# fpgasystems/GPU-FPGA-Recommendation-System

Measured on AMD Instinct MI355X. Metric: inferences/sec at batch 256, higher is better.
Workload: dtype f32; 1 GPU; Model-A (embedding_47_krnl: 47 tables, 1.415 GB) batch=256, fp32 FC 352-1024-512-256-1, all tables resident in one GPU's HBM; hash-filled tables, uniform per-table indices; index rows resident in HBM when the timed region starts (1024 rotating buffers), scores left in HBM (the bench contract's definition of `value`); value_pcie_inclusive = the reference's own loop (cuda_server.c:460-461,494-495): ; batch=256, driver_threads=2, workers_per_thread=2, batches_per_launch=64, parallelism=replicas x1

## Files before the change

### gpu-fpga-recommendation-system_amd/csrc/fr_fused.hip

```cpp
#include "fr_device.h"

constexpr int FR_FT_LD = 33;

template <int NT, int D>
__device__ __forceinline__ void ft_load_a(float4 (&r)[D][NT], const float4 *__restrict__ aq, int N, int g) {
#pragma unroll
    for (int i = 0; i < D; i++)
#pragma unroll
        for (int t = 0; t < NT; t++) r[i][t] = aq[(size_t)(2 * (g + i)) * N + 32 * t];
}

template <int NT, int D>
__device__ __forceinline__ void ft_compute(f32x16 (&acc)[NT], f32x16 &alt, const float4 (&r)[D][NT], const uint4 *bl, int gb) {
    uint4 rb[D];
#pragma unroll
    for (int i = 0; i < D; i++) rb[i] = bl[(size_t)(2 * (gb + i)) * FR_FT_LD];
    __builtin_amdgcn_sched_barrier(0);
#pragma unroll
    for (int i = 0; i < D; i++) {
        const float bx = __uint_as_float(rb[i].x), by = __uint_as_float(rb[i].y), bz = __uint_as_float(rb[i].z), bw = __uint_as_float(rb[i].w);
        if constexpr (NT == 1) {
            acc[0] = __builtin_amdgcn_mfma_f32_32x32x2f32(r[i][0].x, bx, acc[0], 0, 0, 0);
            alt = __builtin_amdgcn_mfma_f32_32x32x2f32(r[i][0].y, by, alt, 0, 0, 0);
            acc[0] = __builtin_amdgcn_mfma_f32_32x32x2f32(r[i][0].z, bz, acc[0], 0, 0, 0);
            alt = __builtin_amdgcn_mfma_f32_32x32x2f32(r[i][0].w, bw, alt, 0, 0, 0);
        } else {
#pragma unroll
            for (int t = 0; t < NT; t++) acc[t] = __builtin_amdgcn_mfma_f32_32x32x2f32(r[i][t].x, bx, acc[t], 0, 0, 0);
#pragma unroll
            for (int t = 0; t < NT; t++) acc[t] = __builtin_amdgcn_mfma_f32_32x32x2f32(r[i][t].y, by, acc[t], 0, 0, 0);
#pragma unroll
            for (int t = 0; t < NT; t++) acc[t] = __builtin_amdgcn_mfma_f32_32x32x2f32(r[i][t].z, bz, acc[t], 0, 0, 0);
#pragma unroll
            for (int t = 0; t < NT; t++) acc[t] = __builtin_amdgcn_mfma_f32_32x32x2f32(r[i][t].w, bw, acc[t], 0, 0, 0);
        }
    }
    __builtin_amdgcn_sched_barrier(0);
}

struct FtW {
    __amdgpu_buffer_rsrc_t rs;
    unsigned voff;
    unsigned row2;
};
__device__ __forceinline__ FtW ft_w(const float4 *wq, int K, int N, int hk, int lm) {
    FtW w;
    w.rs = __builtin_amdgcn_make_buffer_rsrc(const_cast<float4 *>(wq), 0, (unsigned)(K / 4) * (unsigned)N * 16u, 0x00020000);
    w.voff = (unsigned)(hk * N + lm) * 16u;
    w.row2 = 2u * (unsigned)N * 16u;
    return w;
}
__device__ __forceinline__ float4 ft_wload(const FtW &w, unsigned soff, int imm) {
    const u32x4 v = __builtin_amdgcn_raw_buffer_load_b128(w.rs, w.voff + imm, soff, 0);
    return make_float4(__uint_as_float(v.x), __uint_as_float(v.y), __uint_as_float(v.z), __uint_as_float(v.w));
}

template <int NT, int R, int CNT>
__device__ __forceinline__ void ft_ring_fill(float4 (&ring)[R][NT], const FtW &w, int n0, int g0) {
    const unsigned s0 = (unsigned)g0 * w.row2 + (unsigned)n0 * 16u;
#pragma unroll
    for (int g = 0; g < R && g < CNT; g++)
#pragma unroll
        for (int t = 0; t < NT; t++) ring[g][t] = ft_wload(w, s0 + (unsigned)g * w.row2, 512 * t);
    __builtin_amdgcn_sched_barrier(0);
}

template <int NT, int R, int CNT>
__device__ __forceinline__ void ft_gemm_ct(f32x16 (&acc)[NT], float4 (&ring)[R][NT], const FtW &w, int n0, const uint4 *Bq, int gb0, int g0, int hk,
                                           int lm) {
    const unsigned s0 = (unsigned)g0 * w.row2 + (unsigned)n0 * 16u;
    unsigned so = s0 + (unsigned)R * w.row2;
    const uint4 *bl = Bq + (size_t)(2 * gb0 + hk) * FR_FT_LD + lm;
    f32x16 alt;
#pragma unroll
    for (int i = 0; i < 16; i++) alt[i] = 0.0f;
    uint4 bcur = bl[0];
#pragma unroll
    for (int g = 0; g < CNT; g++) {
        const uint4 bnext = bl[(size_t)(2 * ((g + 1 < CNT) ? g + 1 : g)) * FR_FT_LD];
        const float bx = __uint_as_float(bcur.x), by = __uint_as_float(bcur.y), bz = __uint_as_float(bcur.z), bw = __uint_as_float(bcur.w);
        const float4(&a4)[NT] = ring[g % R];
        if constexpr (NT == 1) {
            acc[0] = __builtin_amdgcn_mfma_f32_32x32x2f32(a4[0].x, bx, acc[0], 0, 0, 0);
            alt = __builtin_amdgcn_mfma_f32_32x32x2f32(a4[0].y, by, alt, 0, 0, 0);
            acc[0] = __builtin_amdgcn_mfma_f32_32x32x2f32(a4[0].z, bz, acc[0], 0, 0, 0);
            alt = __builtin_amdgcn_mfma_f32_32x32x2f32(a4[0].w, bw, alt, 0, 0, 0);
        } else {
#pragma unroll
            for (int t = 0; t < NT; t++) acc[t] = __builtin_amdgcn_mfma_f32_32x32x2f32(a4[t].x, bx, acc[t], 0, 0, 0);
#pragma unroll
            for (int t = 0; t < NT; t++) acc[t] = __builtin_amdgcn_mfma_f32_32x32x2f32(a4[t].y, by, acc[t], 0, 0, 0);
#pragma unroll
            for (int t = 0; t < NT; t++) acc[t] = __builtin_amdgcn_mfma_f32_32x32x2f32(a4[t].z, bz, acc[t], 0, 0, 0);
#pragma unroll
            for (int t = 0; t < NT; t++) acc[t] = __builtin_amdgcn_mfma_f32_32x32x2f32(a4[t].w, bw, acc[t], 0, 0, 0);
        }
        if (g + R < CNT) {
#pragma unroll
            for (int t = 0; t < NT; t++) ring[g % R][t] = ft_wload(w, so, 512 * t);
            so += w.row2;
            asm volatile("" : "+s"(so));
        }
        __builtin_amdgcn_sched_barrier(0);
        bcur = bnext;
    }
    if constexpr (NT == 1) {
#pragma unroll
        for (int i = 0; i < 16; i++) acc[0][i] += alt[i];
    }
}

template <int NT, int D>
__device__ __forceinline__ void ft_gemm(f32x16 (&acc)[NT], const float4 *__restrict__ wq, int N, int n0, const uint4 *Bq, int gb0, int g0,
                                        int cnt, int hk, int lm) {
    const float4 *aq = wq + (size_t)hk * N + n0 + lm;
    const uint4 *bl = Bq + hk * FR_FT_LD + lm;
    float4 ra[D][NT], na[D][NT];
    f32x16 alt;
#pragma unroll
    for (int i = 0; i < 16; i++) alt[i] = 0.0f;
    const int nblk = cnt / D;
    ft_load_a<NT, D>(ra, aq, N, g0);
    for (int blk = 0; blk < nblk; blk++) {
        const int nx = (blk + 1 < nblk) ? (blk + 1) : blk;
        ft_load_a<NT, D>(na, aq, N, g0 + nx * D);
        ft_compute<NT, D>(acc, alt, ra, bl, gb0 + blk * D);
#pragma unroll
        for (int i = 0; i < D; i++)
#pragma unroll
            for (int t = 0; t < NT; t++) ra[i][t] = na[i][t];
    }
    if constexpr (NT == 1) {
#pragma unroll
        for (int i = 0; i < 16; i++) acc[0][i] += alt[i];
    }
}

__device__ __forceinline__ void ft_store_tile(uint4 *img, const f32x16 &acc, int n_local, int hk, int lm) {
#pragma unroll
    for (int i = 0; i < 4; i++) {
        uint4 v;
        v.x = __float_as_uint(acc[4 * i + 0]);
        v.y = __float_as_uint(acc[4 * i + 1]);
        v.z = __float_as_uint(acc[4 * i + 2]);
        v.w = __float_as_uint(acc[4 * i + 3]);
        img[(size_t)((n_local >> 2) + 2 * i + hk) * FR_FT_LD + lm] = v;
    }
}

template <int NB, int IPT, typename Sink>
__device__ __forceinline__ bool ft_gather_tile(const FrFusedArgs &a, const FrFusedBatch &bt, int m0, int wl, int ig, Sink &&sink) {
    uint64_t base[NB];
    uint32_t stride[NB], rows[NB], icol[NB];
    bool dense[NB];
#pragma unroll
    for (int p = 0; p < NB; p++) {
        const int w = 64 * p + wl < a.n_words ? 64 * p + wl : a.n_words - 1;
        const uint4 d0 = reinterpret_cast<const uint4 *>(a.words)[2 * w];
        const uint4 d1 = reinterpret_cast<const uint4 *>(a.words)[2 * w + 1];
        dense[p] = (d0.w & FR_DESC_DENSE) != 0;
        base[p] = (dense[p] ? (uint64_t)reinterpret_cast<uintptr_t>(bt.dense) : 0ull) + (((uint64_t)d0.y << 32) | d0.x);
        stride[p] = d0.z, rows[p] = d1.x, icol[p] = dense[p] ? 0u : d0.w * 4u;
    }
    const __amdgpu_buffer_rsrc_t rs_idx = __builtin_amdgcn_make_buffer_rsrc(const_cast<int32_t *>(bt.idx), 0, (unsigned)bt.batch * (unsigned)a.idx_stride * 4u, 0x00020000);
    uint32_t id[NB][IPT];
#pragma unroll
    for (int p = 0; p < NB; p++)
#pragma unroll
        for (int i = 0; i < IPT; i++)
            id[p][i] = (uint32_t)__builtin_amdgcn_raw_buffer_load_b32(rs_idx, (unsigned)(m0 + IPT * ig + i) * (unsigned)a.idx_stride * 4u + icol[p], 0, 0);
    bool bad = false;
    uint4 v[NB][IPT];
    auto load_rows = [&](int p) {
#pragma unroll
        for (int i = 0; i < IPT; i++) {
            const unsigned m = (unsigned)(m0 + IPT * ig + i);
            uint32_t r = id[p][i];
            const bool oob = !dense[p] & (r >= rows[p]);
            bad |= oob;
            r = oob ? 0u : r;
            r = dense[p] ? (m < (unsigned)bt.batch ? m : 0u) : r;
            typedef const u32x4_t __attribute__((address_space(1))) * gptr_t;
            const u32x4_t q = *(gptr_t)(base[p] + (uint64_t)r * stride[p]);
            v[p][i] = make_uint4(q.x, q.y, q.z, q.w);
        }
    };
    load_rows(0);
#pragma unroll
    for (int p = 0; p < NB; p++) {
        if (p + 1 < NB) load_rows(p + 1);
        const int w = 64 * p + wl;
        if (w < a.n_words) {
#pragma unroll
            for (int i = 0; i < IPT; i++) sink(w, i, (m0 + IPT * ig + i < bt.batch) ? v[p][i] : make_uint4(0u, 0u, 0u, 0u));
        }
    }
    return bad;
}

template <int T2W, int KG, int WPE, bool DB>
__global__ void __launch_bounds__(512, WPE) fr_fused_tile_kernel(const FrFusedArgs a) {
    extern __shared__ uint4 lds[];
    constexpr int RD = (WPE == 2) ? 1 : 2;
    const int KQ = a.K / 4;
    uint4 *Xq = lds;
    uint4 *R1b[2] = {Xq + (size_t)KQ * FR_FT_LD, Xq + (size_t)(KQ + (DB ? 64 : 0)) * FR_FT_LD};
    uint4 *R2 = lds;
    uint4 *R3 = DB ? lds + (size_t)(a.H2 / 4) * FR_FT_LD : lds;
    const int tid = threadIdx.x, lane = tid & 63;
    const int wave = __builtin_amdgcn_readfirstlane(tid >> 6);
    const int hk = lane >> 5, lm = lane & 31;
    const int bi = blockIdx.x / a.tiles_per_batch, tile = blockIdx.x - bi * a.tiles_per_batch;
    const FrFusedBatch &bt = a.b[bi];
    const int m0 = tile * 32;
    if (m0 >= bt.batch) return;
    int n_st = 0;
    auto stamp = [&]() {
        if (a.stamps && tid == 0 && n_st < 14) {
            a.stamps[16ull * blockIdx.x + n_st] = __builtin_amdgcn_s_memrealtime();
            if (n_st == 1) a.stamps[16ull * blockIdx.x + 14] = __builtin_amdgcn_s_memtime();
            if (n_st == 11) a.stamps[16ull * blockIdx.x + 15] = __builtin_amdgcn_s_memtime();
        }
        n_st++;
    };
    auto wstamp = [&](int k) {
        if (a.stamps && lane == 0) a.stamps[16ull * gridDim.x + (8ull * blockIdx.x + wave) * 4 + k] = __builtin_amdgcn_s_memrealtime();
    };
    stamp();
    const FtW W1 = ft_w(a.w1q, a.K, a.H1, hk, lm), W2 = ft_w(a.w2q, a.H1, a.H2, hk, lm), W3 = ft_w(a.w3q, a.H2, a.H3, hk, lm);
    constexpr int RA = 16 / RD, RB = 24 / T2W / RD;
    constexpr int KG1 = KG > 0 ? KG : 1;
    float4 ring1[RA][1];
    if constexpr (KG > 0) ft_ring_fill<1, RA, KG1>(ring1, W1, 32 * wave, 0);

    if constexpr (KG > 0) {
        const int wl = tid & 63, ig = tid >> 6;
        constexpr int NB = (2 * KG1 + 63) / 64;
        const bool bad = ft_gather_tile<NB, 4>(a, bt, m0, wl, ig, [&](int w, int i, const uint4 &x) { Xq[(size_t)w * FR_FT_LD + 4 * ig + i] = x; });
        if (bad) atomicOr_system(a.err_flag, 1);
    } else {
        const int wl = tid & 63, ig = tid >> 6;
        bool bad = false;
        for (int w0 = 0; w0 < a.n_words; w0 += 64) {
            const int w = w0 + wl;
            if (w < a.n_words) {
                const uint4 d0 = reinterpret_cast<const uint4 *>(a.words)[2 * w];
                const uint4 d1 = reinterpret_cast<const uint4 *>(a.words)[2 * w + 1];
                const uint64_t src = ((uint64_t)d0.y << 32) | d0.x;
                const uint32_t stride = d0.z, idx_col = d0.w, rows = d1.x;
                const bool is_dense = (idx_col & FR_DESC_DENSE) != 0;
                const char *base = is_dense ? reinterpret_cast<const char *>(bt.dense) + src : reinterpret_cast<const char *>(src);
                uint32_t id[4];
#pragma unroll
                for (int i = 0; i < 4; i++) {
                    const int m = m0 + 4 * ig + i;
                    id[i] = 0;
                    if (m < bt.batch) id[i] = is_dense ? (uint32_t)m : (uint32_t)bt.idx[(size_t)m * a.idx_stride + idx_col];
                    if (!is_dense && id[i] >= rows) {
                        bad = true;
                        id[i] = 0;
                    }
                }
                uint4 v[4];
#pragma unroll
                for (int i = 0; i < 4; i++) v[i] = *reinterpret_cast<const uint4 *>(base + (uint64_t)id[i] * stride);
#pragma unroll
                for (int i = 0; i < 4; i++)
                    Xq[(size_t)w * FR_FT_LD + 4 * ig + i] = (m0 + 4 * ig + i < bt.batch) ? v[i] : make_uint4(0u, 0u, 0u, 0u);
            }
        }
        if (bad) atomicOr_system(a.err_flag, 1);
    }
    __syncthreads();
    stamp();

    f32x16 acc2[T2W];
#pragma unroll
    for (int t = 0; t < T2W; t++)
#pragma unroll
        for (int i = 0; i < 16; i++) acc2[t][i] = 0.0f;
    const int n_chunks = a.H1 / 256;
    for (int c = 0; c < n_chunks; c++) {
        f32x16 acc1[1];
#pragma unroll
        for (int i = 0; i < 16; i++) acc1[0][i] = 0.0f;
        if constexpr (KG > 0) ft_gemm_ct<1, RA, KG1>(acc1, ring1, W1, c * 256 + 32 * wave, Xq, 0, 0, hk, lm);
        else ft_gemm<1, 4>(acc1, a.w1q, a.H1, c * 256 + 32 * wave, Xq, 0, 0, a.K / 8, hk, lm);
        stamp();
        if (c == 1) wstamp(0);
        if (c == 2) wstamp(3);
        float4 ring2[RB][T2W];
        ft_ring_fill<T2W, RB, 32>(ring2, W2, 32 * T2W * wave, 32 * c);
        uint4 *R1 = R1b[c & 1];
        if (!DB && c > 0) __syncthreads();
        ft_store_tile(R1, acc1[0], 32 * wave, hk, lm);
        __syncthreads();
        stamp();
        if (c == 1) wstamp(1);
        ft_gemm_ct<T2W, RB, 32>(acc2, ring2, W2, 32 * T2W * wave, R1, 0, 32 * c, hk, lm);
        if (c == 1) wstamp(2);
        if constexpr (KG > 0) {
            const int cn = (c + 1 < n_chunks) ? c + 1 : c;
            ft_ring_fill<1, RA, KG1>(ring1, W1, cn * 256 + 32 * wave, 0);
        }
    }
    float4 ring3[RA][1];
    ft_ring_fill<1, RA, 32 * T2W>(ring3, W3, 32 * wave, 0);
    __syncthreads();
#pragma unroll
    for (int t = 0; t < T2W; t++) ft_store_tile(R2, acc2[t], 32 * (T2W * wave + t), hk, lm);
    __syncthreads();
    stamp();

    f32x16 acc3[1];
#pragma unroll
    for (int i = 0; i < 16; i++) acc3[0][i] = 0.0f;
    ft_gemm_ct<1, RA, 32 * T2W>(acc3, ring3, W3, 32 * wave, R2, 0, 0, hk, lm);
    if (!DB) __syncthreads();
    ft_store_tile(R3, acc3[0], 32 * wave, hk, lm);
    __syncthreads();
    stamp();
    {
        const int il = tid & 31, sl = tid >> 5;
        const int rows_per = (a.H3 / 4) / 16;
        float s = 0.0f;
        for (int q = sl * rows_per; q < (sl + 1) * rows_per; q++) {
            const uint4 r = R3[(size_t)q * FR_FT_LD + il];
            const float4 w4 = reinterpret_cast<const float4 *>(a.wout)[q];
            s = fmaf(w4.x, __uint_as_float(r.x), s);
            s = fmaf(w4.y, __uint_as_float(r.y), s);
            s = fmaf(w4.z, __uint_as_float(r.z), s);
            s = fmaf(w4.w, __uint_as_float(r.w), s);
        }
        float *part = reinterpret_cast<float *>(R3 + (size_t)64 * FR_FT_LD);
        part[sl * 32 + il] = s;
        __syncthreads();
        if (tid < 32 && m0 + tid < bt.batch) {
            float t = part[tid];
#pragma unroll
            for (int i = 1; i < 16; i++) t += part[i * 32 + tid];
            bt.scores[m0 + tid] = t;
        }
    }
    stamp();
}

size_t frk_fused_lds_bytes(int K, int H2, int wpe) {
    if (wpe == 4) {
        const size_t phase1 = (size_t)(K / 4) + 64, phase2 = (size_t)(H2 / 4) > 68 ? (size_t)(H2 / 4) : 68;
        return (phase1 > phase2 ? phase1 : phase2) * FR_FT_LD * 16;
    }
    const size_t phase1 = (size_t)(K / 4) + 128;
    const size_t phase2 = (size_t)(H2 / 4) + 64 + 4;
    return (phase1 > phase2 ? phase1 : phase2) * FR_FT_LD * 16;
}

bool frk_fused_ok(int K, int H1, int H2, int H3) {
    const bool straight = (K == 352 || K == 880) && H2 == 512;
    if ((!straight && K % 32) || H1 % 256 || (H2 != 256 && H2 != 512) || H3 != 256) return false;
    return frk_fused_lds_bytes(K, H2, 4) <= 160 * 1024;
}

static int fused_wpe(int K, int H2) {
#ifdef FR_EXPERIMENTS
    const int forced = FR_KNOB_ONCE("FUSED_WPE", 0);
    if (forced == 2 || forced == 4) return forced == 4 && frk_fused_lds_bytes(K, H2, 4) > 80 * 1024 ? 2 : forced;
#endif
    return frk_fused_lds_bytes(K, H2, 4) <= 80 * 1024 ? 4 : 2;
}

template <int T2W, int KG, int WPE, bool DB>
static int fused_launch_inst(const FrFusedArgs &a, dim3 grid, size_t lds, hipStream_t s) {
    static FrLdsAttrOnce lds_once;
    if (int rc_ = fr_allow_full_lds(&fr_fused_tile_kernel<T2W, KG, WPE, DB>, lds_once)) return rc_;
    fr_fused_tile_kernel<T2W, KG, WPE, DB><<<grid, dim3(512), lds, s>>>(a);
    fr_note_kernel("fr_fused_tile_kernel<%d, %d, %d, %s>", T2W, KG, WPE, DB ? "true" : "false");
    KCHECK();
    return FR_OK;
}

int frk_fused_launch(const FrFusedArgs &a, hipStream_t s) {
    int wpe = fused_wpe(a.K, a.H2);
    const bool db = wpe == 2 && frk_fused_lds_bytes(a.K, a.H2, 2) <= 160 * 1024;
    const size_t lds = frk_fused_lds_bytes(a.K, a.H2, db ? 2 : 4);
    dim3 grid(a.n_batches * a.tiles_per_batch);
    if (a.H2 == 512) {
        if (a.K == 352) {
#ifdef FR_EXPERIMENTS
            if (wpe != 4) return fused_launch_inst<2, 44, 2, true>(a, grid, lds, s);
#endif
            return fused_launch_inst<2, 44, 4, false>(a, grid, lds, s);
        }
        if (a.K == 880) return fused_launch_inst<2, 110, 2, false>(a, grid, lds, s);
        if (db) return fused_launch_inst<2, 0, 2, true>(a, grid, lds, s);
        return fused_launch_inst<2, 0, 2, false>(a, grid, lds, s);
    }
    if (db) return fused_launch_inst<1, 0, 2, true>(a, grid, lds, s);
    return fused_launch_inst<1, 0, 2, false>(a, grid, lds, s);
}

constexpr int FR_M2_LD = 65;

template <int NT, int MT, int R, int CNT>
__device__ __forceinline__ void ftm_gemm_ct(f32x16 (&acc)[NT][MT], float4 (&ring)[R][NT], const FtW &w, int n0, const uint4 *Bq, int gb0, int g0, int hk,
                                            int lm) {
    const unsigned s0 = (unsigned)g0 * w.row2 + (unsigned)n0 * 16u;
    const uint4 *bl = Bq + (size_t)(2 * gb0 + hk) * FR_M2_LD + lm;
    uint4 bcur[MT];
#pragma unroll
    for (int mt = 0; mt < MT; mt++) bcur[mt] = bl[32 * mt];
    f32x16 alt[MT];
    if constexpr (NT == 1) {
#pragma unroll
        for (int mt = 0; mt < MT; mt++)
#pragma unroll
            for (int i = 0; i < 16; i++) alt[mt][i] = 0.0f;
    }
#pragma unroll
    for (int g = 0; g < CNT; g++) {
        uint4 bnext[MT];
        const int gn = (g + 1 < CNT) ? g + 1 : g;
#pragma unroll
        for (int mt = 0; mt < MT; mt++) bnext[mt] = bl[(size_t)(2 * gn) * FR_M2_LD + 32 * mt];
        const float4(&a4)[NT] = ring[g % R];
#pragma unroll
        for (int c = 0; c < 4; c++)
#pragma unroll
            for (int t = 0; t < NT; t++)
#pragma unroll
                for (int mt = 0; mt < MT; mt++) {
                    const float av = c == 0 ? a4[t].x : c == 1 ? a4[t].y : c == 2 ? a4[t].z : a4[t].w;
                    const uint32_t bv = c == 0 ? bcur[mt].x : c == 1 ? bcur[mt].y : c == 2 ? bcur[mt].z : bcur[mt].w;
                    if (NT == 1 && (c & 1)) alt[mt] = __builtin_amdgcn_mfma_f32_32x32x2f32(av, __uint_as_float(bv), alt[mt], 0, 0, 0);
                    else acc[t][mt] = __builtin_amdgcn_mfma_f32_32x32x2f32(av, __uint_as_float(bv), acc[t][mt], 0, 0, 0);
                }
        if (g + R < CNT) {
#pragma unroll
            for (int t = 0; t < NT; t++) ring[g % R][t] = ft_wload(w, s0 + (unsigned)(g + R) * w.row2, 512 * t);
        }
        __builtin_amdgcn_sched_barrier(0);
#pragma unroll
        for (int mt = 0; mt < MT; mt++) bcur[mt] = bnext[mt];
    }
    if constexpr (NT == 1) {
#pragma unroll
        for (int mt = 0; mt < MT; mt++)
#pragma unroll
            for (int i = 0; i < 16; i++) acc[0][mt][i] += alt[mt][i];
    }
}

__device__ __forceinline__ void ftm_store_tile(uint4 *img, const f32x16 &acc, int n_local, int m_local, int hk, int lm) {
#pragma unroll
    for (int i = 0; i < 4; i++) {
        uint4 v;
        v.x = __float_as_uint(acc[4 * i + 0]);
        v.y = __float_as_uint(acc[4 * i + 1]);
        v.z = __float_as_uint(acc[4 * i + 2]);
        v.w = __float_as_uint(acc[4 * i + 3]);
        img[(size_t)((n_local >> 2) + 2 * i + hk) * FR_M2_LD + m_local + lm] = v;
    }
}

template <int KG>
__global__ void __launch_bounds__(512) fr_fused_tile_m2_kernel(const FrFusedArgs a) {
    extern __shared__ uint4 lds[];
    constexpr int LD = FR_M2_LD, MT = 2, T2W = 2, TI = 64;
    constexpr int RA = 12, RB = 8;
    const int KQ = a.K / 4;
    uint4 *Xq = lds;
    uint4 *R1 = Xq + (size_t)KQ * LD;
    uint4 *R2 = lds;
    uint4 *R3 = lds;
    const int tid = threadIdx.x, lane = tid & 63;
    const int wave = __builtin_amdgcn_readfirstlane(tid >> 6);
    const int hk = lane >> 5, lm = lane & 31;
    const int bi = blockIdx.x / a.tiles_per_batch, tile = blockIdx.x - bi * a.tiles_per_batch;
    const FrFusedBatch &bt = a.b[bi];
    const int m0 = tile * TI;
    if (m0 >= bt.batch) return;
    const FtW W1 = ft_w(a.w1q, a.K, a.H1, hk, lm), W2 = ft_w(a.w2q, a.H1, a.H2, hk, lm), W3 = ft_w(a.w3q, a.H2, a.H3, hk, lm);
    float4 ring1[RA][1];
    ft_ring_fill<1, RA, KG>(ring1, W1, 32 * wave, 0);

    {
        const int wl = tid & 63, ig = tid >> 6;
        constexpr int NB = (2 * KG + 63) / 64;
        const bool bad = ft_gather_tile<NB, 8>(a, bt, m0, wl, ig, [&](int w, int i, const uint4 &x) { Xq[(size_t)w * LD + 8 * ig + i] = x; });
        if (bad) atomicOr_system(a.err_flag, 1);
    }
    __syncthreads();

    f32x16 acc2[T2W][MT];
#pragma unroll
    for (int t = 0; t < T2W; t++)
#pragma unroll
        for (int mt = 0; mt < MT; mt++)
#pragma unroll
            for (int i = 0; i < 16; i++) acc2[t][mt][i] = 0.0f;
    const int n_chunks = a.H1 / 256;
    for (int c = 0; c < n_chunks; c++) {
        f32x16 acc1[1][MT];
#pragma unroll
        for (int mt = 0; mt < MT; mt++)
#pragma unroll
            for (int i = 0; i < 16; i++) acc1[0][mt][i] = 0.0f;
        ftm_gemm_ct<1, MT, RA, KG>(acc1, ring1, W1, c * 256 + 32 * wave, Xq, 0, 0, hk, lm);
        float4 ring2[RB][T2W];
        ft_ring_fill<T2W, RB, 32>(ring2, W2, 32 * T2W * wave, 32 * c);
        if (c > 0) __syncthreads();
#pragma unroll
        for (int mt = 0; mt < MT; mt++) ftm_store_tile(R1, acc1[0][mt], 32 * wave, 32 * mt, hk, lm);
        __syncthreads();
        ftm_gemm_ct<T2W, MT, RB, 32>(acc2, ring2, W2, 32 * T2W * wave, R1, 0, 32 * c, hk, lm);
        const int cn = (c + 1 < n_chunks) ? c + 1 : c;
        ft_ring_fill<1, RA, KG>(ring1, W1, cn * 256 + 32 * wave, 0);
    }
    float4 ring3[RA][1];
    ft_ring_fill<1, RA, 32 * T2W>(ring3, W3, 32 * wave, 0);
    __syncthreads();
#pragma unroll
    for (int t = 0; t < T2W; t++)
#pragma unroll
        for (int mt = 0; mt < MT; mt++) ftm_store_tile(R2, acc2[t][mt], 32 * (T2W * wave + t), 32 * mt, hk, lm);
    __syncthreads();

    f32x16 acc3[1][MT];
#pragma unroll
    for (int mt = 0; mt < MT; mt++)
#pragma unroll
        for (int i = 0; i < 16; i++) acc3[0][mt][i] = 0.0f;
    ftm_gemm_ct<1, MT, RA, 32 * T2W>(acc3, ring3, W3, 32 * wave, R2, 0, 0, hk, lm);
    __syncthreads();
#pragma unroll
    for (int mt = 0; mt < MT; mt++) ftm_store_tile(R3, acc3[0][mt], 32 * wave, 32 * mt, hk, lm);
    __syncthreads();
    {
        const int il = tid & 63, sg = tid >> 6;
        const int rows_per = (a.H3 / 4) / 16;
        float *part = reinterpret_cast<float *>(R3 + (size_t)(a.H3 / 4) * LD);
#pragma unroll
        for (int h2 = 0; h2 < 2; h2++) {
            const int sl = 2 * sg + h2;
            float s = 0.0f;
            for (int q = sl * rows_per; q < (sl + 1) * rows_per; q++) {
                const uint4 r = R3[(size_t)q * LD + il];
                const float4 w4 = reinterpret_cast<const float4 *>(a.wout)[q];
                s = fmaf(w4.x, __uint_as_float(r.x), s);
                s = fmaf(w4.y, __uint_as_float(r.y), s);
                s = fmaf(w4.z, __uint_as_float(r.z), s);
                s = fmaf(w4.w, __uint_as_float(r.w), s);
            }
            part[sl * 64 + il] = s;
        }
        __syncthreads();
        if (tid < 64 && m0 + tid < bt.batch) {
            float t = part[tid];
#pragma unroll
            for (int i = 1; i < 16; i++) t += part[i * 64 + tid];
            bt.scores[m0 + tid] = t;
        }
    }
}

bool frk_fused_m2_ok(int K, int H1, int H2, int H3) { return K == 352 && H1 % 256 == 0 && H2 == 512 && H3 == 256; }

int frk_fused_m2_launch(const FrFusedArgs &a, hipStream_t s) {
    static FrLdsAttrOnce lds_once;
    if (int rc_ = fr_allow_full_lds(&fr_fused_tile_m2_kernel<44>, lds_once)) return rc_;
    const size_t rows1 = (size_t)(a.K / 4) + 64, rows2 = (size_t)(a.H2 / 4), rows3 = 64 + 4;
    const size_t rows = rows1 > rows2 ? (rows1 > rows3 ? rows1 : rows3) : (rows2 > rows3 ? rows2 : rows3);
    fr_fused_tile_m2_kernel<44><<<dim3(a.n_batches * a.tiles_per_batch), dim3(512), rows * FR_M2_LD * 16, s>>>(a);
    fr_note_kernel("fr_fused_tile_m2_kernel<44>");
    KCHECK();
    return FR_OK;
}

template <int NT, int MT, int R, int CNT>
__device__ __forceinline__ void fth_gemm_ct(f32x16 (&acc)[NT][MT], const FtW &w, int n0, const uint4 *Bh, int ld, int gb0, int g0, int hk, int lm) {
    const unsigned s0 = (unsigned)g0 * w.row2 + (unsigned)n0 * 16u;
    const uint4 *bl = Bh + (size_t)(2 * gb0 + hk) * ld + lm;
    uint4 ring[R][NT];
#pragma unroll
    for (int g = 0; g < R && g < CNT; g++)
#pragma unroll
        for (int t = 0; t < NT; t++) ring[g][t] = __builtin_bit_cast(uint4, ft_wload(w, s0 + (unsigned)g * w.row2, 512 * t));
#pragma unroll
    for (int g = 0; g < CNT; g++) {
        uint4 b8[MT];
#pragma unroll
        for (int mt = 0; mt < MT; mt++) b8[mt] = bl[(size_t)(2 * g) * ld + 32 * mt];
#pragma unroll
        for (int t = 0; t < NT; t++)
#pragma unroll
            for (int mt = 0; mt < MT; mt++)
                acc[t][mt] = __builtin_amdgcn_mfma_f32_32x32x16_bf16(__builtin_bit_cast(bf16x8, ring[g % R][t]), __builtin_bit_cast(bf16x8, b8[mt]),
                                                                     acc[t][mt], 0, 0, 0);
        if (g + R < CNT) {
#pragma unroll
            for (int t = 0; t < NT; t++) ring[g % R][t] = __builtin_bit_cast(uint4, ft_wload(w, s0 + (unsigned)(g + R) * w.row2, 512 * t));
        }
        __builtin_amdgcn_sched_barrier(0);
    }
}

__device__ __forceinline__ void fth_store_tile(uint4 *img, int ld, const f32x16 &acc, int n_local, int m_local, int hk, int lm) {
    uint2 *h = reinterpret_cast<uint2 *>(img);
#pragma unroll
    for (int i = 0; i < 4; i++) {
        uint2 v;
        v.x = pack_bf16x2(acc[4 * i + 0], acc[4 * i + 1]);
        v.y = pack_bf16x2(acc[4 * i + 2], acc[4 * i + 3]);
        h[((size_t)((n_local >> 3) + i) * ld + m_local + lm) * 2 + hk] = v;
    }
}

template <int MT, int T2W, int KG, bool DB, int RD, int PD>
__global__ void __launch_bounds__(512) fr_fused_tile_h_kernel(const FrFusedArgs a) {
    extern __shared__ uint4 lds[];
    constexpr int LD = 32 * MT + 1, TI = 32 * MT;
    const int KO = a.K / 8;
    uint4 *Xh = lds;
    uint4 *R1b[2] = {Xh + (size_t)KO * LD, Xh + (size_t)(KO + (DB ? 32 : 0)) * LD};
    uint4 *R2 = lds;
    uint4 *R3 = lds + (size_t)(a.H2 / 8) * LD;
    const int tid = threadIdx.x, lane = tid & 63;
    const int wave = __builtin_amdgcn_readfirstlane(tid >> 6);
    const int hk = lane >> 5, lm = lane & 31;
    const int bi = blockIdx.x / a.tiles_per_batch, tile = blockIdx.x - bi * a.tiles_per_batch;
    const FrFusedBatch &bt = a.b[bi];
    const int m0 = tile * TI;
    if (m0 >= bt.batch) return;
    int n_st = 0;
    auto stamp = [&]() {
        if (a.stamps && lane == 0 && n_st < 14) {
            a.stamps[16ull * (8ull * blockIdx.x + wave) + n_st] = __builtin_amdgcn_s_memrealtime();
            if (n_st == 1) a.stamps[16ull * (8ull * blockIdx.x + wave) + 14] = __builtin_amdgcn_s_memtime();
            if (n_st == 9) a.stamps[16ull * (8ull * blockIdx.x + wave) + 15] = __builtin_amdgcn_s_memtime();
        }
        n_st++;
    };
    stamp();

    {
        const int wl = tid & 63, ig = tid >> 6;
        constexpr int IPT = TI / 8, NB = (4 * KG + 63) / 64;
        uint2 *Xh2 = reinterpret_cast<uint2 *>(Xh);
        const bool bad = ft_gather_tile<NB, IPT>(a, bt, m0, wl, ig, [&](int w, int i, const uint4 &x) {
            uint2 hv;
            hv.x = pack_bf16x2(__uint_as_float(x.x), __uint_as_float(x.y));
            hv.y = pack_bf16x2(__uint_as_float(x.z), __uint_as_float(x.w));
            Xh2[((size_t)(w >> 1) * LD + IPT * ig + i) * 2 + (w & 1)] = hv;
        });
        if (bad) atomicOr_system(a.err_flag, 1);
    }
    __syncthreads();
    stamp();

    f32x16 acc2[T2W][MT];
#pragma unroll
    for (int t = 0; t < T2W; t++)
#pragma unroll
        for (int mt = 0; mt < MT; mt++)
#pragma unroll
            for (int i = 0; i < 16; i++) acc2[t][mt][i] = 0.0f;
    const int n_chunks = a.H1 / 256;
    const FtW W1 = ft_w(a.w1q, a.K / 2, a.H1, hk, lm), W2 = ft_w(a.w2q, a.H1 / 2, a.H2, hk, lm), W3 = ft_w(a.w3q, a.H2 / 2, a.H3, hk, lm);
    static_assert(T2W == 2 && KG >= RD && RD >= 8 && RD <= 32 && RD % 2 == 0, "the stream ring assumes two n tiles per wave in FC2 (32 elements per chunk) and at least RD k groups in FC1");
    constexpr int OFF2 = KG % RD;
    uint4 ring[RD];
    auto w1load = [&](int c, int g) { return __builtin_bit_cast(uint4, ft_wload(W1, (unsigned)g * W1.row2 + (unsigned)(c * 256 + 32 * wave) * 16u, 0)); };
    auto w2load = [&](int c, int e) {
        return __builtin_bit_cast(uint4, ft_wload(W2, (unsigned)(16 * c + (e >> 1)) * W2.row2 + (unsigned)(32 * T2W * wave) * 16u, 512 * (e & 1)));
    };
#pragma unroll
    for (int g = 0; g < RD; g++) ring[g] = w1load(0, g);
    const uint4 *blx = Xh + (size_t)hk * LD + lm;
    static_assert(PD == 1 || PD == 2 || PD == 4, "B ring: 16 % PD must be 0");
    uint4 bq[PD][MT];
#pragma unroll
    for (int i = 0; i < PD; i++)
#pragma unroll
        for (int mt = 0; mt < MT; mt++) bq[i][mt] = blx[(size_t)(2 * i) * LD + 32 * mt];
    for (int c = 0; c < n_chunks; c++) {
        f32x16 acc1[1][MT];
#pragma unroll
        for (int mt = 0; mt < MT; mt++)
#pragma unroll
            for (int i = 0; i < 16; i++) acc1[0][mt][i] = 0.0f;
#pragma unroll
        for (int g = 0; g < KG; g++) {
#pragma unroll
            for (int mt = 0; mt < MT; mt++)
                acc1[0][mt] = __builtin_amdgcn_mfma_f32_32x32x16_bf16(__builtin_bit_cast(bf16x8, ring[g % RD]), __builtin_bit_cast(bf16x8, bq[g % PD][mt]), acc1[0][mt], 0, 0, 0);
            if (g + PD < KG) {
#pragma unroll
                for (int mt = 0; mt < MT; mt++) bq[g % PD][mt] = blx[(size_t)(2 * (g + PD)) * LD + 32 * mt];
            }
            if (g + RD < KG) ring[g % RD] = w1load(c, g + RD);
            else ring[g % RD] = w2load(c, (g % RD - OFF2 + RD) % RD);
            __builtin_amdgcn_sched_barrier(0);
        }
        stamp();
        uint4 *R1 = R1b[DB ? (c & 1) : 0];
        if (!DB && c > 0) __syncthreads();
#pragma unroll
        for (int mt = 0; mt < MT; mt++) fth_store_tile(R1, LD, acc1[0][mt], 32 * wave, 32 * mt, hk, lm);
        __syncthreads();
        const bool last = c + 1 == n_chunks;
        FtW WN = W1;
        if (last) WN = W3;
        const unsigned nsoff = last ? (unsigned)(32 * wave) * 16u : (unsigned)((c + 1) * 256 + 32 * wave) * 16u;
        const uint4 *blr = R1 + (size_t)hk * LD + lm;
#pragma unroll
        for (int i = 0; i < PD; i++)
#pragma unroll
            for (int mt = 0; mt < MT; mt++) bq[i][mt] = blr[(size_t)(2 * i) * LD + 32 * mt];
#pragma unroll
        for (int j = 0; j < 16; j++) {
#pragma unroll
            for (int t = 0; t < T2W; t++)
#pragma unroll
                for (int mt = 0; mt < MT; mt++)
                    acc2[t][mt] = __builtin_amdgcn_mfma_f32_32x32x16_bf16(__builtin_bit_cast(bf16x8, ring[(2 * j + t + OFF2) % RD]), __builtin_bit_cast(bf16x8, bq[j % PD][mt]),
                                                                         acc2[t][mt], 0, 0, 0);
#pragma unroll
            for (int mt = 0; mt < MT; mt++)
                bq[j % PD][mt] = j + PD < 16 ? blr[(size_t)(2 * (j + PD)) * LD + 32 * mt] : blx[(size_t)(2 * (j + PD - 16)) * LD + 32 * mt];
#pragma unroll
            for (int t = 0; t < T2W; t++) {
                const int r = (2 * j + t + OFF2) % RD;
                if (2 * j + t + RD < 32) ring[r] = w2load(c, 2 * j + t + RD);
                else ring[r] = __builtin_bit_cast(uint4, ft_wload(WN, (unsigned)r * WN.row2 + nsoff, 0));
            }
            __builtin_amdgcn_sched_barrier(0);
        }
        stamp();
    }
    __syncthreads();
#pragma unroll
    for (int t = 0; t < T2W; t++)
#pragma unroll
        for (int mt = 0; mt < MT; mt++) fth_store_tile(R2, LD, acc2[t][mt], 32 * (T2W * wave + t), 32 * mt, hk, lm);
    __syncthreads();

    f32x16 acc3[1][MT];
#pragma unroll
    for (int mt = 0; mt < MT; mt++)
#pragma unroll
        for (int i = 0; i < 16; i++) acc3[0][mt][i] = 0.0f;
    {
        const uint4 *bl3 = R2 + (size_t)hk * LD + lm;
#pragma unroll
        for (int i = 0; i < PD; i++)
#pragma unroll
            for (int mt = 0; mt < MT; mt++) bq[i][mt] = bl3[(size_t)(2 * i) * LD + 32 * mt];
#pragma unroll
        for (int g = 0; g < 16 * T2W; g++) {
#pragma unroll
            for (int mt = 0; mt < MT; mt++)
                acc3[0][mt] = __builtin_amdgcn_mfma_f32_32x32x16_bf16(__builtin_bit_cast(bf16x8, ring[g % RD]), __builtin_bit_cast(bf16x8, bq[g % PD][mt]), acc3[0][mt], 0, 0, 0);
            if (g + PD < 16 * T2W) {
#pragma unroll
                for (int mt = 0; mt < MT; mt++) bq[g % PD][mt] = bl3[(size_t)(2 * (g + PD)) * LD + 32 * mt];
            }
            if (g + RD < 16 * T2W) ring[g % RD] = __builtin_bit_cast(uint4, ft_wload(W3, (unsigned)(g + RD) * W3.row2 + (unsigned)(32 * wave) * 16u, 0));
            __builtin_amdgcn_sched_barrier(0);
        }
    }
#pragma unroll
    for (int mt = 0; mt < MT; mt++) fth_store_tile(R3, LD, acc3[0][mt], 32 * wave, 32 * mt, hk, lm);
    __syncthreads();
    stamp();
    {
        const int il = tid % TI, sl = tid / TI;
        constexpr int NSL = 512 / TI;
        const int rows_per = (a.H3 / 8) / NSL;
        const uint4 *wh = reinterpret_cast<const uint4 *>(a.wout);
        float s = 0.0f;
        for (int q = sl * rows_per; q < (sl + 1) * rows_per; q++) {
            const uint4 r = R3[(size_t)q * LD + il];
            const uint4 w = wh[q];
            const uint32_t rr[4] = {r.x, r.y, r.z, r.w}, ww[4] = {w.x, w.y, w.z, w.w};
#pragma unroll
            for (int e = 0; e < 4; e++) {
                s = fmaf(__uint_as_float(ww[e] << 16), __uint_as_float(rr[e] << 16), s);
                s = fmaf(__uint_as_float(ww[e] & 0xFFFF0000u), __uint_as_float(rr[e] & 0xFFFF0000u), s);
            }
        }
        float *part = reinterpret_cast<float *>(R3 + (size_t)(a.H3 / 8) * LD);
        part[sl * TI + il] = s;
        __syncthreads();
        if (tid < TI && m0 + tid < bt.batch) {
            float t = part[tid];
#pragma unroll
            for (int i = 1; i < NSL; i++) t += part[i * TI + tid];
            bt.scores[m0 + tid] = t;
        }
    }
}

static size_t fused_h_lds_bytes(int K, int H2, int H3, int MT, bool db) {
    const size_t LD = 32 * MT + 1;
    const size_t phase1 = (size_t)(K / 8) + (db ? 64 : 32);
    const size_t phase2 = (size_t)(H2 / 8) + (size_t)(H3 / 8) + 2;
    return (phase1 > phase2 ? phase1 : phase2) * LD * 16;
}

bool frk_fused_h_ok(int K, int H1, int H2, int H3) {
    if (H1 % 256 || H2 != 512 || H3 != 256) return false;
    return K == 352 || K == 880;
}

int frk_fused_h_items_per_wg() { return 64; }

template <int MT, int T2W, int KG, bool DB, int RD, int PD>
static int fused_h_launch_inst(const FrFusedArgs &a, dim3 grid, size_t lds, hipStream_t s) {
    static FrLdsAttrOnce lds_once;
    if (int rc_ = fr_allow_full_lds(&fr_fused_tile_h_kernel<MT, T2W, KG, DB, RD, PD>, lds_once)) return rc_;
    fr_fused_tile_h_kernel<MT, T2W, KG, DB, RD, PD><<<grid, dim3(512), lds, s>>>(a);
    fr_note_kernel("fr_fused_tile_h_kernel<%d, %d, %d, %s, %d, %d>", MT, T2W, KG, DB ? "true" : "false", RD, PD);
    KCHECK();
    return FR_OK;
}

int frk_fused_h_launch(const FrFusedArgs &a, hipStream_t s) {
    dim3 grid(a.n_batches * a.tiles_per_batch);
    if (a.K == 352) return fused_h_launch_inst<2, 2, 22, true, 16, 2>(a, grid, fused_h_lds_bytes(a.K, a.H2, a.H3, 2, true), s);
    if (a.K == 880) return fused_h_launch_inst<2, 2, 55, false, 12, 2>(a, grid, fused_h_lds_bytes(a.K, a.H2, a.H3, 2, false), s);
    FR_FAIL(FR_ERR_INVALID, "no bf16 fused instantiation for K=%d", a.K);
}

struct FtW8 {
    __amdgpu_buffer_rsrc_t rs;
    unsigned voff, voff2;
    unsigned grp;
};
__device__ __forceinline__ FtW8 ft_w8(const void *wf, int KE, int N, int hk, int lm) {
    FtW8 w;
    w.rs = __builtin_amdgcn_make_buffer_rsrc(const_cast<void *>(wf), 0, (unsigned)KE * (unsigned)N * 16u, 0x00020000);
    w.voff = ((unsigned)(2 * hk) * N + lm) * 16u;
    w.voff2 = w.voff + (unsigned)N * 16u;
    w.grp = 4u * (unsigned)N * 16u;
    return w;
}
__device__ __forceinline__ i32x8 ft_w8load(const FtW8 &w, unsigned soff, int imm) {
    const u32x4 lo = __builtin_amdgcn_raw_buffer_load_b128(w.rs, w.voff + imm, soff, 0), hi = __builtin_amdgcn_raw_buffer_load_b128(w.rs, w.voff2 + imm, soff, 0);
    i32x8 r;
    r[0] = (int)lo.x; r[1] = (int)lo.y; r[2] = (int)lo.z; r[3] = (int)lo.w;
    r[4] = (int)hi.x; r[5] = (int)hi.y; r[6] = (int)hi.z; r[7] = (int)hi.w;
    return r;
}

template <int NT, int MT, int R, int CNT>
__device__ __forceinline__ void ft8_gemm_ct(f32x16 (&acc)[NT][MT], const FtW8 &w, int n0, const uint4 *Bf, int ld, int gb0, int g0, int hk, int lm, int sc_a,
                                            int sc_b) {
    const unsigned s0 = (unsigned)g0 * w.grp + (unsigned)n0 * 16u;
    const uint4 *bl = Bf + (size_t)(4 * gb0 + 2 * hk) * ld + lm;
    i32x8 ring[R][NT];
#pragma unroll
    for (int g = 0; g < R && g < CNT; g++)
#pragma unroll
        for (int t = 0; t < NT; t++) ring[g][t] = ft_w8load(w, s0 + (unsigned)g * w.grp, 512 * t);
#pragma unroll
    for (int g = 0; g < CNT; g++) {
        i32x8 b8[MT];
#pragma unroll
        for (int mt = 0; mt < MT; mt++) {
            const uint4 lo = bl[(size_t)(4 * g) * ld + 32 * mt], hi = bl[(size_t)(4 * g + 1) * ld + 32 * mt];
            b8[mt][0] = (int)lo.x; b8[mt][1] = (int)lo.y; b8[mt][2] = (int)lo.z; b8[mt][3] = (int)lo.w;
            b8[mt][4] = (int)hi.x; b8[mt][5] = (int)hi.y; b8[mt][6] = (int)hi.z; b8[mt][7] = (int)hi.w;
        }
#pragma unroll
        for (int t = 0; t < NT; t++)
#pragma unroll
            for (int mt = 0; mt < MT; mt++) acc[t][mt] = __builtin_amdgcn_mfma_scale_f32_32x32x64_f8f6f4(ring[g % R][t], b8[mt], acc[t][mt], 0, 0, 0, sc_a, 0, sc_b);
        if (g + R < CNT) {
#pragma unroll
            for (int t = 0; t < NT; t++) ring[g % R][t] = ft_w8load(w, s0 + (unsigned)(g + R) * w.grp, 512 * t);
        }
        __builtin_amdgcn_sched_barrier(0);
    }
}

__device__ __forceinline__ void ft8_store_tile(uint4 *img, int ld, const f32x16 &acc, int n_local, int m_local, int hk, int lm, float oscale) {
    uint32_t *q = reinterpret_cast<uint32_t *>(img);
#pragma unroll
    for (int i = 0; i < 4; i++) {
        const int n = n_local + 8 * i + 4 * hk;
        q[((size_t)(n >> 4) * ld + m_local + lm) * 4 + ((n & 15) >> 2)] = pack_fp8x4(acc[4 * i + 0], acc[4 * i + 1], acc[4 * i + 2], acc[4 * i + 3], oscale);
    }
}

template <int G1 >
__global__ void __launch_bounds__(512) fr_fused_tile_f8_kernel(const FrFusedArgs a) {
    extern __shared__ uint4 lds[];
    constexpr int MT = 2, T2W = 2, LD = 32 * MT + 1, TI = 32 * MT;
    constexpr int KE1 = 4 * G1;
    uint4 *Xf = lds;
    uint4 *R1b[2] = {Xf + (size_t)KE1 * LD, Xf + (size_t)(KE1 + 16) * LD};
    uint4 *R2 = lds;
    uint4 *R3 = lds + (size_t)(a.H2 / 16) * LD;
    const int tid = threadIdx.x, lane = tid & 63;
    const int wave = __builtin_amdgcn_readfirstlane(tid >> 6);
    const int hk = lane >> 5, lm = lane & 31;
    const int bi = blockIdx.x / a.tiles_per_batch, tile = blockIdx.x - bi * a.tiles_per_batch;
    const FrFusedBatch &bt = a.b[bi];
    const int m0 = tile * TI;
    if (m0 >= bt.batch) return;

    {
        const int wl = tid & 63, ig = tid >> 6;
        uint32_t *Xw = reinterpret_cast<uint32_t *>(Xf);
        const float scale = __builtin_ldexpf(1.0f, a.e_act[0]);
        constexpr int NB = (4 * KE1 + 63) / 64;
        const bool bad = ft_gather_tile<NB, 8>(a, bt, m0, wl, ig, [&](int w, int i, const uint4 &x) {
            Xw[((size_t)(w >> 2) * LD + 8 * ig + i) * 4 + (w & 3)] = pack_fp8_word(x, scale);
        });
        for (int w = a.n_words + tid; w < 4 * KE1; w += 512)
#pragma unroll 1
            for (int i = 0; i < TI; i++) Xw[((size_t)(w >> 2) * LD + i) * 4 + (w & 3)] = 0u;
        if (bad) atomicOr_system(a.err_flag, 1);
    }
    __syncthreads();

    f32x16 acc2[T2W][MT];
#pragma unroll
    for (int t = 0; t < T2W; t++)
#pragma unroll
        for (int mt = 0; mt < MT; mt++)
#pragma unroll
            for (int i = 0; i < 16; i++) acc2[t][mt][i] = 0.0f;
    const int n_chunks = a.H1 / 256;
    const FtW8 W1 = ft_w8(a.w1q, KE1, a.H1, hk, lm), W2 = ft_w8(a.w2q, a.H1 / 16, a.H2, hk, lm), W3 = ft_w8(a.w3q, a.H2 / 16, a.H3, hk, lm);
    const float os1 = __builtin_ldexpf(1.0f, a.e_act[1]), os2 = __builtin_ldexpf(1.0f, a.e_act[2]), os3 = __builtin_ldexpf(1.0f, a.e_act[3]);
    for (int c = 0; c < n_chunks; c++) {
        f32x16 acc1[1][MT];
#pragma unroll
        for (int mt = 0; mt < MT; mt++)
#pragma unroll
            for (int i = 0; i < 16; i++) acc1[0][mt][i] = 0.0f;
        ft8_gemm_ct<1, MT, (G1 < 8 ? G1 : 8), G1>(acc1, W1, c * 256 + 32 * wave, Xf, LD, 0, 0, hk, lm, 127 - a.e_w[0], 127 - a.e_act[0]);
        uint4 *R1 = R1b[c & 1];
#pragma unroll
        for (int mt = 0; mt < MT; mt++) ft8_store_tile(R1, LD, acc1[0][mt], 32 * wave, 32 * mt, hk, lm, os1);
        __syncthreads();
        ft8_gemm_ct<T2W, MT, 4, 4>(acc2, W2, 32 * T2W * wave, R1, LD, 0, 4 * c, hk, lm, 127 - a.e_w[1], 127 - a.e_act[1]);
    }
    __syncthreads();
#pragma unroll
    for (int t = 0; t < T2W; t++)
#pragma unroll
        for (int mt = 0; mt < MT; mt++) ft8_store_tile(R2, LD, acc2[t][mt], 32 * (T2W * wave + t), 32 * mt, hk, lm, os2);
    __syncthreads();

    f32x16 acc3[1][MT];
#pragma unroll
    for (int mt = 0; mt < MT; mt++)
#pragma unroll
        for (int i = 0; i < 16; i++) acc3[0][mt][i] = 0.0f;
    ft8_gemm_ct<1, MT, 8, 8>(acc3, W3, 32 * wave, R2, LD, 0, 0, hk, lm, 127 - a.e_w[2], 127 - a.e_act[2]);
#pragma unroll
    for (int mt = 0; mt < MT; mt++) ft8_store_tile(R3, LD, acc3[0][mt], 32 * wave, 32 * mt, hk, lm, os3);
    __syncthreads();
    {
        const int il = tid & 63, sl = tid >> 6;
        const int rows_per = (a.H3 / 16) / 8;
        float s = 0.0f;
        for (int q = sl * rows_per; q < (sl + 1) * rows_per; q++) {
            const uint4 r = R3[(size_t)q * LD + il];
            const int rr[4] = {(int)r.x, (int)r.y, (int)r.z, (int)r.w};
            const float *w = a.wout + 16 * q;
#pragma unroll
            for (int c = 0; c < 4; c++) {
                s = fmaf(w[4 * c + 0], __builtin_amdgcn_cvt_f32_fp8(rr[c], 0), s);
                s = fmaf(w[4 * c + 1], __builtin_amdgcn_cvt_f32_fp8(rr[c], 1), s);
                s = fmaf(w[4 * c + 2], __builtin_amdgcn_cvt_f32_fp8(rr[c], 2), s);
                s = fmaf(w[4 * c + 3], __builtin_amdgcn_cvt_f32_fp8(rr[c], 3), s);
            }
        }
        float *part = reinterpret_cast<float *>(R3 + (size_t)(a.H3 / 16) * LD);
        part[sl * 64 + il] = s;
        __syncthreads();
        if (tid < 64 && m0 + tid < bt.batch) {
            float t = part[tid];
#pragma unroll
            for (int i = 1; i < 8; i++) t += part[i * 64 + tid];
            bt.scores[m0 + tid] = t * __builtin_ldexpf(1.0f, -a.e_act[3]);
        }
    }
}

bool frk_fused_f8_ok(int K, int H1, int H2, int H3) { return (K == 352 || K == 880) && H1 % 256 == 0 && H2 == 512 && H3 == 256; }

template <int G1>
static int fused_f8_launch_inst(const FrFusedArgs &a, hipStream_t s) {
    static FrLdsAttrOnce lds_once;
    if (int rc_ = fr_allow_full_lds(&fr_fused_tile_f8_kernel<G1>, lds_once)) return rc_;
    const size_t rows1 = 4 * G1 + 32, rows2 = (size_t)(a.H2 / 16) + (size_t)(a.H3 / 16) + 2;
    fr_fused_tile_f8_kernel<G1><<<dim3(a.n_batches * a.tiles_per_batch), dim3(512), (rows1 > rows2 ? rows1 : rows2) * 65 * 16, s>>>(a);
    fr_note_kernel("fr_fused_tile_f8_kernel<%d>", G1);
    KCHECK();
    return FR_OK;
}

int frk_fused_f8_launch(const FrFusedArgs &a, hipStream_t s) {
    if (a.K == 352) return fused_f8_launch_inst<6>(a, s);
    if (a.K == 880) return fused_f8_launch_inst<14>(a, s);
    FR_FAIL(FR_ERR_INVALID, "no fp8 fused instantiation for K=%d", a.K);
}
```

Baseline: 69.12 million inferences/s.

## Overlap embedding gather with first-layer GEMM via staged slices in fused m2 kernel

Splits the embedding gather for the first FC layer into four word slices. Each slice's row loads are issued up front and stored to LDS just before its part of the chunk-0 layer-1 GEMM runs, so HBM gather latency overlaps with MFMA work instead of finishing behind a single barrier. It also adds a deeper weight ring for chunk 0, split acc/alt accumulators, and optional timestamp probes compiled only under FR_EXPERIMENTS. The cost is extra barriers and higher register pressure from holding all slice rows and the larger ring, which may reduce occupancy or cause spills.

```diff
diff --git a/gpu-fpga-recommendation-system_amd/csrc/fr_fused.hip b/gpu-fpga-recommendation-system_amd/csrc/fr_fused.hip
--- a/gpu-fpga-recommendation-system_amd/csrc/fr_fused.hip
+++ b/gpu-fpga-recommendation-system_amd/csrc/fr_fused.hip
@@ -462,6 +462,78 @@
     }
 }
 
+template <int MT, int R, int CNT, int GA, int GB>
+__device__ __forceinline__ void ftm_gemm_part(f32x16 (&acc)[MT], f32x16 (&alt)[MT], float4 (&ring)[R][1], const FtW &w, unsigned s0, const uint4 *bl) {
+    uint4 bcur[MT];
+#pragma unroll
+    for (int mt = 0; mt < MT; mt++) bcur[mt] = bl[(size_t)(2 * GA) * FR_M2_LD + 32 * mt];
+#pragma unroll
+    for (int g = GA; g < GB; g++) {
+        uint4 bnext[MT];
+        const int gn = (g + 1 < GB) ? g + 1 : g;
+#pragma unroll
+        for (int mt = 0; mt < MT; mt++) bnext[mt] = bl[(size_t)(2 * gn) * FR_M2_LD + 32 * mt];
+        const float4 a4 = ring[g % R][0];
+#pragma unroll
+        for (int c = 0; c < 4; c++)
+#pragma unroll
+            for (int mt = 0; mt < MT; mt++) {
+                const float av = c == 0 ? a4.x : c == 1 ? a4.y : c == 2 ? a4.z : a4.w;
+                const uint32_t bv = c == 0 ? bcur[mt].x : c == 1 ? bcur[mt].y : c == 2 ? bcur[mt].z : bcur[mt].w;
+                if (c & 1) alt[mt] = __builtin_amdgcn_mfma_f32_32x32x2f32(av, __uint_as_float(bv), alt[mt], 0, 0, 0);
+                else acc[mt] = __builtin_amdgcn_mfma_f32_32x32x2f32(av, __uint_as_float(bv), acc[mt], 0, 0, 0);
+            }
+        if (g + R < CNT) ring[g % R][0] = ft_wload(w, s0 + (unsigned)(g + R) * w.row2, 0);
+        __builtin_amdgcn_sched_barrier(0);
+#pragma unroll
+        for (int mt = 0; mt < MT; mt++) bcur[mt] = bnext[mt];
+    }
+}
+
+template <int S0, int W>
+struct FtmSlice {
+    static constexpr int IPT = W / 8;
+    int w, mi;
+    uint64_t base;
+    uint32_t stride, rows, icol;
+    bool dense;
+    uint32_t id[IPT];
+    uint4 v[IPT];
+    __device__ __forceinline__ void descriptor(const FrFusedArgs &a, const FrFusedBatch &bt, int m0, int lane, int wave) {
+        w = S0 + (lane & (W - 1));
+        mi = m0 + 8 * wave + IPT * (lane / W);
+        const uint4 d0 = reinterpret_cast<const uint4 *>(a.words)[2 * w];
+        const uint4 d1 = reinterpret_cast<const uint4 *>(a.words)[2 * w + 1];
+        dense = (d0.w & FR_DESC_DENSE) != 0;
+        base = (dense ? (uint64_t)reinterpret_cast<uintptr_t>(bt.dense) : 0ull) + (((uint64_t)d0.y << 32) | d0.x);
+        stride = d0.z, rows = d1.x, icol = dense ? 0u : d0.w * 4u;
+    }
+    __device__ __forceinline__ void indices(const FrFusedArgs &a, __amdgpu_buffer_rsrc_t rs_idx) {
+#pragma unroll
+        for (int i = 0; i < IPT; i++) id[i] = (uint32_t)__builtin_amdgcn_raw_buffer_load_b32(rs_idx, (unsigned)(mi + i) * (unsigned)a.idx_stride * 4u + icol, 0, 0);
+    }
+    __device__ __forceinline__ bool row_loads(const FrFusedBatch &bt) {
+        bool bad = false;
+#pragma unroll
+        for (int i = 0; i < IPT; i++) {
+            const unsigned m = (unsigned)(mi + i);
+            uint32_t r = id[i];
+            const bool oob = !dense & (r >= rows);
+            bad |= oob;
+            r = oob ? 0u : r;
+            r = dense ? (m < (unsigned)bt.batch ? m : 0u) : r;
+            typedef const u32x4_t __attribute__((address_space(1))) * gptr_t;
+            const u32x4_t q = *(gptr_t)(base + (uint64_t)r * stride);
+            v[i] = make_uint4(q.x, q.y, q.z, q.w);
+        }
+        return bad;
+    }
+    __device__ __forceinline__ void store(uint4 *Xq, const FrFusedBatch &bt, int m0) const {
+#pragma unroll
+        for (int i = 0; i < IPT; i++) Xq[(size_t)w * FR_M2_LD + (mi - m0) + i] = (mi + i < bt.batch) ? v[i] : make_uint4(0u, 0u, 0u, 0u);
+    }
+};
+
 template <int KG>
 __global__ void __launch_bounds__(512) fr_fused_tile_m2_kernel(const FrFusedArgs a) {
     extern __shared__ uint4 lds[];
@@ -480,16 +552,65 @@
     const int m0 = tile * TI;
     if (m0 >= bt.batch) return;
     const FtW W1 = ft_w(a.w1q, a.K, a.H1, hk, lm), W2 = ft_w(a.w2q, a.H1, a.H2, hk, lm), W3 = ft_w(a.w3q, a.H2, a.H3, hk, lm);
-    float4 ring1[RA][1];
-    ft_ring_fill<1, RA, KG>(ring1, W1, 32 * wave, 0);
-
-    {
-        const int wl = tid & 63, ig = tid >> 6;
-        constexpr int NB = (2 * KG + 63) / 64;
-        const bool bad = ft_gather_tile<NB, 8>(a, bt, m0, wl, ig, [&](int w, int i, const uint4 &x) { Xq[(size_t)w * LD + 8 * ig + i] = x; });
-        if (bad) atomicOr_system(a.err_flag, 1);
-    }
-    __syncthreads();
+#ifdef FR_EXPERIMENTS
+    int n_st = 0;
+    auto stamp = [&]() {
+        if (a.stamps && tid == 0) a.stamps[16ull * blockIdx.x + n_st] = __builtin_amdgcn_s_memrealtime();
+        n_st++;
+    };
+#else
+    auto stamp = [] {};
+#endif
+    stamp();
+
+    static_assert(KG == 44, "the slices below cover 88 record words");
+    constexpr int R0 = 20;
+    float4 ring0[R0][1];
+    ft_ring_fill<1, R0, KG>(ring0, W1, 32 * wave, 0);
+    FtmSlice<0, 8> sl0;
+    FtmSlice<8, 16> sl1;
+    FtmSlice<24, 32> sl2;
+    FtmSlice<56, 32> sl3;
+    sl0.descriptor(a, bt, m0, lane, wave), sl1.descriptor(a, bt, m0, lane, wave), sl2.descriptor(a, bt, m0, lane, wave), sl3.descriptor(a, bt, m0, lane, wave);
+    __builtin_amdgcn_sched_barrier(0);
+    const __amdgpu_buffer_rsrc_t rs_idx = __builtin_amdgcn_make_buffer_rsrc(const_cast<int32_t *>(bt.idx), 0, (unsigned)bt.batch * (unsigned)a.idx_stride * 4u, 0x00020000);
+    sl0.indices(a, rs_idx), sl1.indices(a, rs_idx), sl2.indices(a, rs_idx), sl3.indices(a, rs_idx);
+    __builtin_amdgcn_sched_barrier(0);
+    bool bad = sl0.row_loads(bt);
+    bad |= sl1.row_loads(bt);
+    bad |= sl2.row_loads(bt);
+    bad |= sl3.row_loads(bt);
+    __builtin_amdgcn_sched_barrier(0);
+
+    f32x16 acc1[1][MT], alt1[MT];
+#pragma unroll
+    for (int mt = 0; mt < MT; mt++)
+#pragma unroll
+        for (int i = 0; i < 16; i++) acc1[0][mt][i] = 0.0f, alt1[mt][i] = 0.0f;
+    const unsigned s1 = (unsigned)(32 * wave) * 16u;
+    const uint4 *bl1 = Xq + (size_t)hk * LD + lm;
+    sl0.store(Xq, bt, m0);
+    __syncthreads();
+    stamp();
+    ftm_gemm_part<MT, R0, KG, 0, 4>(acc1[0], alt1, ring0, W1, s1, bl1);
+    sl1.store(Xq, bt, m0);
+    __syncthreads();
+    stamp();
+    ftm_gemm_part<MT, R0, KG, 4, 12>(acc1[0], alt1, ring0, W1, s1, bl1);
+    sl2.store(Xq, bt, m0);
+    __syncthreads();
+    stamp();
+    ftm_gemm_part<MT, R0, KG, 12, 28>(acc1[0], alt1, ring0, W1, s1, bl1);
+    sl3.store(Xq, bt, m0);
+    __syncthreads();
+    stamp();
+    ftm_gemm_part<MT, R0, KG, 28, 44>(acc1[0], alt1, ring0, W1, s1, bl1);
+#pragma unroll
+    for (int mt = 0; mt < MT; mt++)
+#pragma unroll
+        for (int i = 0; i < 16; i++) acc1[0][mt][i] += alt1[mt][i];
+    stamp();
+    if (bad) atomicOr_system(a.err_flag, 1);
 
     f32x16 acc2[T2W][MT];
 #pragma unroll
@@ -499,13 +620,8 @@
 #pragma unroll
             for (int i = 0; i < 16; i++) acc2[t][mt][i] = 0.0f;
     const int n_chunks = a.H1 / 256;
-    for (int c = 0; c < n_chunks; c++) {
-        f32x16 acc1[1][MT];
-#pragma unroll
-        for (int mt = 0; mt < MT; mt++)
-#pragma unroll
-            for (int i = 0; i < 16; i++) acc1[0][mt][i] = 0.0f;
-        ftm_gemm_ct<1, MT, RA, KG>(acc1, ring1, W1, c * 256 + 32 * wave, Xq, 0, 0, hk, lm);
+    float4 ring1[RA][1];
+    auto chunk_tail = [&](int c) __attribute__((always_inline)) {
         float4 ring2[RB][T2W];
         ft_ring_fill<T2W, RB, 32>(ring2, W2, 32 * T2W * wave, 32 * c);
         if (c > 0) __syncthreads();
@@ -515,6 +631,15 @@
         ftm_gemm_ct<T2W, MT, RB, 32>(acc2, ring2, W2, 32 * T2W * wave, R1, 0, 32 * c, hk, lm);
         const int cn = (c + 1 < n_chunks) ? c + 1 : c;
         ft_ring_fill<1, RA, KG>(ring1, W1, cn * 256 + 32 * wave, 0);
+    };
+    chunk_tail(0);
+    for (int c = 1; c < n_chunks; c++) {
+#pragma unroll
+        for (int mt = 0; mt < MT; mt++)
+#pragma unroll
+            for (int i = 0; i < 16; i++) acc1[0][mt][i] = 0.0f;
+        ftm_gemm_ct<1, MT, RA, KG>(acc1, ring1, W1, c * 256 + 32 * wave, Xq, 0, 0, hk, lm);
+        chunk_tail(c);
     }
     float4 ring3[RA][1];
     ft_ring_fill<1, RA, 32 * T2W>(ring3, W3, 32 * wave, 0);
@@ -535,6 +660,7 @@
 #pragma unroll
     for (int mt = 0; mt < MT; mt++) ftm_store_tile(R3, acc3[0][mt], 32 * wave, 32 * mt, hk, lm);
     __syncthreads();
+    stamp();
     {
         const int il = tid & 63, sg = tid >> 6;
         const int rows_per = (a.H3 / 4) / 16;
@@ -561,6 +687,7 @@
             bt.scores[m0 + tid] = t;
         }
     }
+    stamp();
 }
 
 bool frk_fused_m2_ok(int K, int H1, int H2, int H3) { return K == 352 && H1 % 256 == 0 && H2 == 512 && H3 == 256; }
```

Result: no change. 68.52 million inferences/s (-0.9%).
